# thethomasboyer/PhenDiff

Measured on NVIDIA B200. Metric: images/sec, DDIM invert+regenerate 128x128 100 steps, higher is better.
Workload: dtype fp16

## Files before the change

include/phendiff_b200.h:

```cpp
#ifndef PHENDIFF_B200_H
#define PHENDIFF_B200_H

#include <stddef.h>
#include <stdint.h>

#ifdef __cplusplus
extern "C" {
#endif

typedef struct pd_unet pd_unet_t;
typedef struct pd_train pd_train_t;
typedef void* pd_stream_t;

enum { PD_PREC_FP32 = 0, PD_PREC_BF16 = 1, PD_PREC_FP16 = 2 };
enum { PD_PRED_EPSILON = 0, PD_PRED_SAMPLE = 1, PD_PRED_V = 2 };
#define PD_MAX_BLOCKS 8

typedef struct pd_unet_config {
    int32_t in_channels;
    int32_t out_channels;
    int32_t n_blocks;
    int32_t block_out_channels[PD_MAX_BLOCKS];
    int32_t down_attn[PD_MAX_BLOCKS];
    int32_t up_attn[PD_MAX_BLOCKS];
// ... 76 lines not shown
                       pd_stream_t stream);
int pd_train_launch_count(pd_train_t* t, int64_t* n);

int pd_train_forward(pd_train_t* t, const float* params, const float* x, const float* timesteps, const int64_t* labels, float* model_out,
                     pd_stream_t stream);
int pd_train_backward_input(pd_train_t* t, const float* d_model_out, float* d_input, pd_stream_t stream);
int pd_guidance_lp_grad(const pd_step_coeffs_t* step, const float* x, const float* model_out, const float* ref, int32_t batch, int64_t per,
                        float p, float* scratch, float* losses, float* d_model_out, float* d_x, pd_stream_t stream);
#define PD_ADAMW_SCRATCH_FLOATS 1185
int pd_adamw_step(float* params, const float* grads, float* exp_avg, float* exp_avg_sq, float* ema, int64_t n, float lr, float beta1,
                  float beta2, float eps, float weight_decay, int32_t step, float max_grad_norm, float ema_decay, float* scratch,
                  float* grad_norm_out, pd_stream_t stream);

int pd_unet_launch_count(pd_unet_t* h, int64_t* n);
int pd_unet_plan_info(pd_unet_t* h, int32_t* microbatch, int32_t* tc_layers, int32_t* simt_layers, int32_t* ops);

enum { PD_CLS_CONV_TC = 0, PD_CLS_CONV_SIMT, PD_CLS_GN, PD_CLS_ATTN, PD_CLS_EMBED, PD_CLS_CONV_IN, PD_CLS_CONV_OUT,
       PD_CLS_UPSAMPLE, PD_CLS_COUNT };
int pd_unet_profile_begin(pd_unet_t* h, int32_t every_n, int32_t max_samples);
int pd_unet_profile_end(pd_unet_t* h, int32_t* samples);
int pd_unet_profile_query(pd_unet_t* h, int32_t cls, double* ms, int64_t* launches, double* flops);
int pd_unet_profile_op(pd_unet_t* h, int32_t idx, const char** name, int32_t* cls, double* ms, int32_t* samples, double* flops);

int pd_test_conv(int32_t use_tc, int32_t dtype, int32_t n, int32_t h, int32_t w, int32_t c1, int32_t c2,
                 int32_t cout, int32_t ksize, int32_t stride, int32_t pad, const void* x1, const void* x2,
                 const float* weight, const float* bias, const float* addvec, const void* residual,
                 const void* sc1, const void* sc2, int32_t csc1, int32_t csc2, const float* sc_w, float out_scale,
                 void* out, pd_stream_t stream);
typedef struct pd_test_conv_args {
    int32_t impl, dtype, n, h, w, c1, c2, cout, ksize, stride, pad, upsample, mode, stats_cw, csc1, csc2;
    const void *x1, *x2;
    const float *weight, *bias, *addvec;
    const int32_t* addvec_row;
    const void* residual;
    const void *sc1, *sc2;
    const float* sc_w;
    float out_scale;
    void* out;
    double* stats_out;
    float* model_out;
    float* x_t;
    const pd_step_coeffs_t* step;
} pd_test_conv_args_t;
int pd_test_conv_ex(const pd_test_conv_args_t* args, pd_stream_t stream);
int pd_test_gn_conv(int32_t dtype, int32_t n, int32_t h, int32_t w, int32_t c1, int32_t c2, int32_t cout, int32_t groups, float eps,
                    const void* x1, const void* x2, const float* gamma, const float* beta, const float* weight, const float* bias,
                    const float* addvec, const void* residual, const void* sc1, const void* sc2, int32_t csc1, int32_t csc2,
                    const float* sc_w, float out_scale, void* out, double* stats_out, pd_stream_t stream);
int pd_test_groupnorm(int32_t dtype, int32_t n, int32_t hw, int32_t c1, int32_t c2, int32_t groups, float eps,
                      int32_t do_silu, const void* x1, const void* x2, const float* gamma, const float* beta,
                      void* out, pd_stream_t stream);
int pd_test_attention(int32_t use_mma, int32_t dtype, int32_t n, int32_t s, int32_t c, int32_t d, const void* qkv,
                      void* out, pd_stream_t stream);

#ifdef __cplusplus
}
#endif
#endif
```

phendiff_b200/_lib.py:

```python
from __future__ import annotations

import ctypes as C
import os
from pathlib import Path

_HERE = Path(__file__).resolve().parent
LIB_PATH = _HERE / "libphendiff_b200.so"

PD_PREC_FP32, PD_PREC_BF16, PD_PREC_FP16 = 0, 1, 2
PD_PRED = {"epsilon": 0, "sample": 1, "v_prediction": 2}
PD_MAX_BLOCKS = 8


class UnetConfig(C.Structure):
    _fields_ = [
        ("in_channels", C.c_int32), ("out_channels", C.c_int32), ("n_blocks", C.c_int32),
        ("block_out_channels", C.c_int32 * PD_MAX_BLOCKS),
        ("down_attn", C.c_int32 * PD_MAX_BLOCKS), ("up_attn", C.c_int32 * PD_MAX_BLOCKS),
        ("layers_per_block", C.c_int32), ("attention_head_dim", C.c_int32), ("norm_num_groups", C.c_int32),
        ("norm_eps", C.c_float), ("num_class_embeds", C.c_int32), ("flip_sin_to_cos", C.c_int32),
        ("freq_shift", C.c_float), ("downsample_padding", C.c_int32), ("mid_block_scale_factor", C.c_float),
        ("add_attention", C.c_int32), ("precision", C.c_int32), ("max_microbatch", C.c_int32),
        ("conv_impl", C.c_int32), ("attn_impl", C.c_int32),
    ]
# ... 13 lines not shown
                + [(n, C.c_void_p) for n in ("x1", "x2", "weight", "bias", "addvec", "addvec_row", "residual", "sc1", "sc2", "sc_w")]
                + [("out_scale", C.c_float)]
                + [(n, C.c_void_p) for n in ("out", "stats_out", "model_out", "x_t", "step")])


_P = C.c_void_p
_SIGNATURES = {
    "pd_last_error": (C.c_char_p, []),
    "pd_version": (C.c_int, []),
    "pd_unet_create": (C.c_int, [C.POINTER(UnetConfig), C.POINTER(_P)]),
    "pd_unet_destroy": (C.c_int, [_P]),
    "pd_unet_num_params": (C.c_int, [_P, C.POINTER(C.c_int32)]),
    "pd_unet_param_info": (C.c_int, [_P, C.c_int32, C.POINTER(C.c_char_p), C.POINTER(C.c_int32), C.POINTER(C.c_int64 * 4)]),
    "pd_unet_load_weight": (C.c_int, [_P, C.c_char_p, _P, C.POINTER(C.c_int64), C.c_int32]),
    "pd_unet_finalize": (C.c_int, [_P, _P]),
    "pd_unet_time_embed_dim": (C.c_int, [_P, C.POINTER(C.c_int32)]),
    "pd_unet_plan": (C.c_int, [_P, C.c_int32, C.c_int32, C.c_int32, C.POINTER(C.c_size_t)]),
    "pd_unet_bind_workspace": (C.c_int, [_P, _P, C.c_size_t]),
    "pd_unet_forward": (C.c_int, [_P, _P, _P, _P, _P, _P, _P]),
    "pd_ddim_step": (C.c_int, [C.POINTER(StepCoeffs), _P, _P, _P, _P, _P, C.c_int64, _P]),
    "pd_axpby_per_sample": (C.c_int, [_P, _P, _P, _P, _P, C.c_int32, C.c_int64, _P]),
    "pd_cfg_combine": (C.c_int, [_P, _P, _P, C.c_int32, _P, C.c_int32, C.c_int64, _P]),
    "pd_denorm_nhwc": (C.c_int, [_P, _P, C.c_int32, C.c_int32, C.c_int32, C.c_int32, _P]),
    "pd_ddib_transfer": (C.c_int, [_P, _P, _P, _P, C.POINTER(StepCoeffs), C.c_int32, C.c_int32, _P]),
    "pd_unet_plan_guided": (C.c_int, [_P, C.c_int32, C.c_int32, C.c_int32, C.POINTER(C.c_size_t)]),
    "pd_cfg_transfer": (C.c_int, [_P, _P, _P, _P, C.c_int32, C.POINTER(StepCoeffs), C.c_int32, _P]),
    "pd_train_create": (C.c_int, [_P, C.c_int32, C.c_int32, C.c_int32, C.POINTER(_P)]),
    "pd_train_destroy": (C.c_int, [_P]),
    "pd_train_set_precision": (C.c_int, [_P, C.c_int32]),
    "pd_train_tc_counts": (C.c_int, [_P, C.POINTER(C.c_int64), C.POINTER(C.c_int64)]),
    "pd_train_num_params_flat": (C.c_int, [_P, C.POINTER(C.c_int64)]),
    "pd_train_param_offset": (C.c_int, [_P, C.c_int32, C.POINTER(C.c_int64)]),
    "pd_train_workspace_bytes": (C.c_int, [_P, C.POINTER(C.c_size_t)]),
    "pd_train_bind": (C.c_int, [_P, _P, C.c_size_t]),
    "pd_train_step_grad": (C.c_int, [_P] * 11),
    "pd_train_launch_count": (C.c_int, [_P, C.POINTER(C.c_int64)]),
    "pd_train_forward": (C.c_int, [_P] * 7),
    "pd_train_backward_input": (C.c_int, [_P] * 4),
    "pd_guidance_lp_grad": (C.c_int, [C.POINTER(StepCoeffs), _P, _P, _P, C.c_int32, C.c_int64, C.c_float, _P, _P, _P, _P, _P]),
    "pd_adamw_step": (C.c_int, [_P, _P, _P, _P, _P, C.c_int64, C.c_float, C.c_float, C.c_float, C.c_float, C.c_float, C.c_int32,
                                 C.c_float, C.c_float, _P, _P, _P]),
    "pd_debug_pair_kernel_launches": (C.c_longlong, []),
    "pd_unet_launch_count": (C.c_int, [_P, C.POINTER(C.c_int64)]),
    "pd_unet_plan_info": (C.c_int, [_P, C.POINTER(C.c_int32), C.POINTER(C.c_int32), C.POINTER(C.c_int32), C.POINTER(C.c_int32)]),
    "pd_unet_profile_begin": (C.c_int, [_P, C.c_int32, C.c_int32]),
    "pd_unet_profile_end": (C.c_int, [_P, C.POINTER(C.c_int32)]),
    "pd_unet_profile_query": (C.c_int, [_P, C.c_int32, C.POINTER(C.c_double), C.POINTER(C.c_int64), C.POINTER(C.c_double)]),
    "pd_unet_profile_op": (C.c_int, [_P, C.c_int32, C.POINTER(C.c_char_p), C.POINTER(C.c_int32), C.POINTER(C.c_double), C.POINTER(C.c_int32), C.POINTER(C.c_double)]),
    "pd_test_conv": (C.c_int, [C.c_int32] * 11 + [_P, _P, _P, _P, _P, _P, _P, _P, C.c_int32, C.c_int32, _P, C.c_float, _P, _P]),
    "pd_test_conv_ex": (C.c_int, [C.POINTER(TestConvArgs), _P]),
    "pd_test_gn_conv": (C.c_int, [C.c_int32] * 8 + [C.c_float] + [_P] * 10 + [C.c_int32, C.c_int32, _P, C.c_float, _P, _P, _P]),
    "pd_test_groupnorm": (C.c_int, [C.c_int32] * 6 + [C.c_float, C.c_int32, _P, _P, _P, _P, _P, _P]),
    "pd_test_attention": (C.c_int, [C.c_int32] * 6 + [_P, _P, _P]),
}

EXPORTED_SYMBOLS = tuple(_SIGNATURES)

_lib = None


class PhenDiffB200Error(RuntimeError):
    pass


def lib():
    global _lib
    if _lib is None:
        path = os.environ.get("PHENDIFF_B200_LIB", str(LIB_PATH))
        if not os.path.exists(path):
            raise PhenDiffB200Error(
                f"{path} not found: build it with `python -c 'import __graft_entry__ as g; g.build()'` "
                "(or phendiff_b200/csrc/build.sh). phendiff_b200 has no CPU or PyTorch fallback.")
        l = C.CDLL(path)
        for name, (res, args) in _SIGNATURES.items():
            fn = getattr(l, name)
            fn.restype = res
            fn.argtypes = args
        _lib = l
    return _lib


def check(rc: int):
    if rc != 0:
        msg = lib().pd_last_error()
        raise PhenDiffB200Error(msg.decode() if msg else f"phendiff_b200 error code {rc}")


def ptr(t):
    return None if t is None else C.c_void_p(t.data_ptr())


def current_stream():
    import torch

    return C.c_void_p(torch.cuda.current_stream().cuda_stream)


def require_cuda(t, what: str):
    if not t.is_cuda:
        raise PhenDiffB200Error(
            f"{what} must be a CUDA tensor: phendiff_b200 is the B200 path and has no CPU fallback (got device {t.device})")
```

phendiff_b200/csrc/pd_api.cu:

```cuda
#include "pd_model.h"

namespace pd {

static thread_local std::string g_err;
void set_error(const std::string& m) { g_err = m; }

}

using namespace pd;


namespace pd {

static Param* add_param(pd_unet* m, const std::string& name, std::vector<int64_t> shape) {
    auto p = std::make_unique<Param>();
    p->name = name;
    p->shape = shape;
    p->numel = 1;
    for (auto s : shape) p->numel *= (size_t)s;
    Param* r = p.get();
    m->by_name[name] = r;
    m->params.push_back(std::move(p));
    return r;
}
// ... 1226 lines not shown
    return rc;
}

int pd_test_conv(int32_t use_tc, int32_t dt, int32_t n, int32_t h, int32_t w, int32_t c1, int32_t c2, int32_t cout,
                 int32_t ksize, int32_t stride, int32_t pad, const void* x1, const void* x2, const float* weight,
                 const float* bias, const float* addvec, const void* residual, const void* sc1, const void* sc2,
                 int32_t csc1, int32_t csc2, const float* sc_w, float out_scale, void* out, pd_stream_t stream) {
    pd_test_conv_args_t a;
    memset(&a, 0, sizeof(a));
    a.impl = use_tc; a.dtype = dt; a.n = n; a.h = h; a.w = w; a.c1 = c1; a.c2 = c2; a.cout = cout; a.ksize = ksize;
    a.stride = stride; a.pad = pad; a.x1 = x1; a.x2 = x2; a.weight = weight; a.bias = bias; a.addvec = addvec;
    a.residual = residual; a.sc1 = sc1; a.sc2 = sc2; a.csc1 = csc1; a.csc2 = csc2; a.sc_w = sc_w; a.out_scale = out_scale;
    a.out = out;
    return pd_test_conv_ex(&a, stream);
}

int pd_test_groupnorm(int32_t dt, int32_t n, int32_t hw, int32_t c1, int32_t c2, int32_t groups, float eps,
                      int32_t do_silu, const void* x1, const void* x2, const float* gamma, const float* beta, void* out,
                      pd_stream_t stream) {
    cudaStream_t s = (cudaStream_t)stream;
    PD_REQUIRE(groups > 0 && (c1 + c2) % groups == 0, "channels not divisible by groups");
    int cw = 4;
    while (cw > 1 && (((c1 + c2) / groups) % cw != 0 || c1 % cw != 0)) cw >>= 1;
    double* stats = nullptr;
    const size_t n1 = (size_t)n * (c1 / cw) * 2, n2 = (size_t)n * (c2 / cw) * 2;
    PD_CHECK_CUDA(cudaMalloc((void**)&stats, (n1 + n2 + 2) * sizeof(double)));
    PD_CHECK_CUDA(cudaMemsetAsync(stats, 0, (n1 + n2 + 2) * sizeof(double), s));
    GNArgs ga{};
    ga.x1 = x1; ga.x2 = x2; ga.C1 = c1; ga.C2 = c2; ga.N = n; ga.HW = hw; ga.groups = groups; ga.eps = eps; ga.gamma = gamma;
    ga.beta = beta; ga.silu = do_silu; ga.stats1 = stats; ga.stats2 = c2 ? stats + n1 : nullptr; ga.stats_cw = cw; ga.out = out;
    int rc = launch_gn_chunk_stats(dt, x1, n, hw, c1, cw, stats, s);
    if (!rc && c2) rc = launch_gn_chunk_stats(dt, x2, n, hw, c2, cw, stats + n1, s);
    if (!rc) rc = launch_gn_apply(dt, dt == 0, ga, s);
    cudaError_t e = cudaStreamSynchronize(s);
    cudaFree(stats);
    if (!rc && e != cudaSuccess) { set_error(std::string("groupnorm kernel failed: ") + cudaGetErrorString(e)); rc = 2; }
    return rc;
}

int pd_test_attention(int32_t use_mma, int32_t dt, int32_t n, int32_t s_len, int32_t c, int32_t d, const void* qkv,
                      void* out, pd_stream_t stream) {
    cudaStream_t s = (cudaStream_t)stream;
    int rc;
    if (use_mma) {
        rc = launch_attention_mma(dt, qkv, n, s_len, c, d, use_mma >= 2 ? PD_ATTN_QFOLD : 1.0f, out, s, use_mma >= 3 ? use_mma - 1 : 0);
    } else {
        rc = launch_attention_simt(dt, dt == 0, qkv, n, s_len, c, d, out, s);
    }
    cudaError_t e = cudaStreamSynchronize(s);
    if (!rc && e != cudaSuccess) { set_error(std::string("attention kernel failed: ") + cudaGetErrorString(e)); rc = 2; }
    return rc;
}

}
```

phendiff_b200/csrc/pd_attn_common.cuh:

```cuda
#pragma once
#include "pd_kernels.h"
#include <type_traits>

namespace pd {

__device__ __forceinline__ float ex2(float x) {
    float y;
    asm("ex2.approx.ftz.f32 %0, %1;" : "=f"(y) : "f"(x));
    return y;
}
__device__ __forceinline__ float ex2_poly(float x) {
    x = fminf(fmaxf(x, -100.0f), 128.0f);
    const float t = x + 12582912.0f;
    const float f = x - (t - 12582912.0f);
    float p = 0.05508868396282196f;
    p = fmaf(p, f, 0.24260404706001282f);
    p = fmaf(p, f, 0.6932762265205383f);
    p = fmaf(p, f, 0.9999289512634277f);
    return __int_as_float(__float_as_int(p) + (__float_as_int(t) << 23));
}
__device__ __forceinline__ uint32_t h2op_add(uint32_t a, uint32_t b) { uint32_t d; asm("add.rn.f16x2 %0, %1, %2;" : "=r"(d) : "r"(a), "r"(b)); return d; }
__device__ __forceinline__ uint32_t h2op_sub(uint32_t a, uint32_t b) { uint32_t d; asm("sub.rn.f16x2 %0, %1, %2;" : "=r"(d) : "r"(a), "r"(b)); return d; }
__device__ __forceinline__ uint32_t h2op_mul(uint32_t a, uint32_t b) { uint32_t d; asm("mul.rn.f16x2 %0, %1, %2;" : "=r"(d) : "r"(a), "r"(b)); return d; }
__device__ __forceinline__ uint32_t h2op_fma(uint32_t a, uint32_t b, uint32_t c) { uint32_t d; asm("fma.rn.f16x2 %0, %1, %2, %3;" : "=r"(d) : "r"(a), "r"(b), "r"(c)); return d; }
__device__ __forceinline__ uint32_t h2op_min(uint32_t a, uint32_t b) { uint32_t d; asm("min.f16x2 %0, %1, %2;" : "=r"(d) : "r"(a), "r"(b)); return d; }
__device__ __forceinline__ uint32_t h2op_max(uint32_t a, uint32_t b) { uint32_t d; asm("max.f16x2 %0, %1, %2;" : "=r"(d) : "r"(a), "r"(b)); return d; }

__device__ __forceinline__ uint32_t ex2_pair_h2(float xa, float xb) {
    uint32_t x = pack_f16x2(xa, xb);
    x = h2op_min(h2op_max(x, 0xCB80CB80u ), 0x4C004C00u );
    const uint32_t w = h2op_add(x, 0x640F640Fu );
    const uint32_t f = h2op_sub(x, h2op_sub(w, 0x640F640Fu));
    uint32_t p = h2op_fma(0x2B0D2B0Du , f, 0x33C333C3u );
    p = h2op_fma(p, f, 0x398C398Cu );
    p = h2op_fma(p, f, 0x3C003C00u );
    return h2op_mul(p, w * 1024u + (0u - 0x64006400u * 1024u));
}

template <typename T> __device__ __forceinline__ uint32_t ex2_pair_poly(float xa, float xb);
template <> __device__ __forceinline__ uint32_t ex2_pair_poly<f16>(float xa, float xb) { return ex2_pair_h2(xa, xb); }
template <> __device__ __forceinline__ uint32_t ex2_pair_poly<bf16>(float xa, float xb) { return pack_bf16x2(ex2_poly(xa), ex2_poly(xb)); }


}
```

phendiff_b200/csrc/pd_attn_mma.cu:

```cuda
#include "pd_attn_common.cuh"

namespace pd {

constexpr int AT_WARPS = 8;
constexpr int AT_MAXS = 1024;

template <typename T>
__device__ __forceinline__ void mma_16x8x8(float c[4], uint32_t a0, uint32_t a1, uint32_t b0) {
    if (std::is_same<T, bf16>::value)
        asm volatile("mma.sync.aligned.m16n8k8.row.col.f32.bf16.bf16.f32 {%0,%1,%2,%3}, {%4,%5}, {%6}, {%0,%1,%2,%3};"
                     : "+f"(c[0]), "+f"(c[1]), "+f"(c[2]), "+f"(c[3])
                     : "r"(a0), "r"(a1), "r"(b0));
    else
        asm volatile("mma.sync.aligned.m16n8k8.row.col.f32.f16.f16.f32 {%0,%1,%2,%3}, {%4,%5}, {%6}, {%0,%1,%2,%3};"
                     : "+f"(c[0]), "+f"(c[1]), "+f"(c[2]), "+f"(c[3])
                     : "r"(a0), "r"(a1), "r"(b0));
}
template <typename T>
__device__ __forceinline__ void mma_16x8x16(float c[4], uint32_t a0, uint32_t a1, uint32_t a2, uint32_t a3, uint32_t b0,
                                            uint32_t b1) {
    if (std::is_same<T, bf16>::value)
        asm volatile(
            "mma.sync.aligned.m16n8k16.row.col.f32.bf16.bf16.f32 {%0,%1,%2,%3}, {%4,%5,%6,%7}, {%8,%9}, {%0,%1,%2,%3};"
            : "+f"(c[0]), "+f"(c[1]), "+f"(c[2]), "+f"(c[3])
// ... 346 lines not shown
    if (variant < 0) {
        const char* e = getenv("PHENDIFF_B200_ATTN_KERNEL");
        variant = !e ? 6 : ((e[0] == 'v' && e[1] == '2') ? 2 : ((e[0] == 't' && e[1] == 'c') ? (e[2] == '3' ? 6 : (e[2] == '2' ? 5 : 4)) : 3));
        const char* pe = getenv("PHENDIFF_B200_ATTN_POLYPAIRS");
        polyv = pe ? atoi(pe) : -1;
    }
    const size_t smem = (size_t)S * 32;
    const int var = force_variant ? force_variant : variant;
    if (var == 2 || smem > 200 * 1024) return launch_attention_chunked(dt, qkv, N, S, C, d, AH_SL / qfold, out, s);
    const bool tc3 = var == 6 && S % 128 == 0 && attention_tc3_supported(S, C) && fabsf(AH_SL / qfold - 1.0f) < 1e-6f;
    if (tc3 || ((var == 4 || var == 5) && S % 128 == 0 && attention_tc_smem_bytes(S) <= 110 * 1024)) {
        static uint8_t* flags_dev[PD_MAX_DEVICES] = {nullptr};
        static size_t flags_cap_dev[PD_MAX_DEVICES] = {0};
        uint8_t*& flags = flags_dev[pd_cur_dev()];
        size_t& flags_cap = flags_cap_dev[pd_cur_dev()];
        const size_t need = (size_t)N * (C / 8) * (S >> 7) * 4;
        if (need > flags_cap) {
            if (flags) PD_CHECK_CUDA(cudaFree(flags));
            PD_CHECK_CUDA(cudaMalloc(&flags, need));
            flags_cap = need;
        }
        const int tc_pp = polyv < 0 ? (dt == DT_F16 ? 4 : 2) : polyv;
        int rc = tc3 ? launch_attention_tc3(dt, qkv, N, S, C, out, flags, tc_pp, s)
                 : (var == 5 ? launch_attention_tc2(dt, qkv, N, S, C, AH_SL / qfold, out, flags, tc_pp, s)
                             : launch_attention_tc(dt, qkv, N, S, C, AH_SL / qfold, out, flags, tc_pp, s));
        if (rc) return rc;
        dim3 grid(1, C / 8, N);
        PD_DISPATCH_HALF(dt, T, (launch_head<T, 0x0000u>(qkv, N, S, C, AH_SL / qfold, out, grid, smem, s, flags)));
        PD_CHECK_CUDA(cudaGetLastError());
        return 0;
    }
    const float qmul = AH_SL / qfold;
    const int heads = C / 8;
    int split = 1;
    while (split < 8 && (size_t)heads * N * split < 1184 && (S >> 4) / (split * 2) >= AH_WARPS) split *= 2;
    dim3 grid(split, heads, N);
    int pp = polyv;
    if (pp < 0) pp = (dt == DT_F16) ? 6 : 4;
#define PD_AH(MASK) PD_DISPATCH_HALF(dt, T, (launch_head<T, MASK>(qkv, N, S, C, qmul, out, grid, smem, s)))
    switch (pp) {
        case 0: PD_AH(0x0000u); break;
        case 4: PD_AH(0x4242u); break;
        case 6: PD_AH(0x6262u); break;
        case 7: PD_AH(0x6662u); break;
        case 10: PD_AH(0xE6E6u); break;
        case 12: PD_AH(0xEEEEu); break;
        default: PD_AH(0x6666u); break;
    }
#undef PD_AH
    PD_CHECK_CUDA(cudaGetLastError());
    return 0;
}

}
```

phendiff_b200/csrc/pd_attn_tc3.cu:

```cuda
#include "pd_attn_common.cuh"
#include "pd_tc_common.cuh"

namespace pd {

constexpr int A3_NWG = 3;
__host__ __device__ constexpr int a3_threads(int sp) { return 128 + 128 * A3_NWG * sp; }
constexpr int A3_TMEM_COLS = 512;
constexpr int A3_WG_COLS = 160;
constexpr int A3_KT = 64;

struct A3Params {
    CUtensorMap tm;
    int S, C, heads, items, tok_box;
    void* out;
    uint8_t* flags;
    int swap_k, swap_mn;
    int nws;
};

__device__ __forceinline__ void a3_mma_ts(uint32_t d_tmem, uint32_t a_tmem, uint64_t b_desc, uint32_t idesc, uint32_t accumulate) {
    asm volatile(
        "{\n\t.reg .pred p;\n\tsetp.ne.b32 p, %4, 0;\n\t"
        "tcgen05.mma.cta_group::1.kind::f16 [%0], [%1], %2, %3, p;\n\t}\n" ::"r"(d_tmem),
        "r"(a_tmem), "l"(b_desc), "r"(idesc), "r"(accumulate)
// ... 8 lines not shown
        : "memory");
}
__device__ __forceinline__ void a3_st_wait() { asm volatile("tcgen05.wait::st.sync.aligned;" ::: "memory"); }
__device__ __forceinline__ void a3_ld_x16(uint32_t taddr, uint32_t (&r)[16]) {
    asm volatile(
        "tcgen05.ld.sync.aligned.32x32b.x16.b32 "
        "{%0, %1, %2, %3, %4, %5, %6, %7, %8, %9, %10, %11, %12, %13, %14, %15}, [%16];"
        : "=r"(r[0]), "=r"(r[1]), "=r"(r[2]), "=r"(r[3]), "=r"(r[4]), "=r"(r[5]), "=r"(r[6]), "=r"(r[7]),
          "=r"(r[8]), "=r"(r[9]), "=r"(r[10]), "=r"(r[11]), "=r"(r[12]), "=r"(r[13]), "=r"(r[14]), "=r"(r[15])
        : "r"(taddr));
}

__device__ __forceinline__ bool a3_try_wait_hint(uint64_t* bar, uint32_t parity, uint32_t ns) {
    uint32_t ok;
    asm volatile(
        "{\n\t.reg .pred P;\n\tmbarrier.try_wait.parity.shared::cta.b64 P, [%1], %2, %3;\n\tselp.b32 %0, 1, 0, P;\n\t}\n"
        : "=r"(ok) : "r"(smem_u32(bar)), "r"(parity), "r"(ns) : "memory");
    return ok != 0;
}
__device__ __forceinline__ void a3_wait(uint64_t* bar, uint32_t parity) {
    if (a3_try_wait_hint(bar, parity, 2000u)) return;
    const long long t0 = clock64();
    for (;;) {
#pragma unroll 1
        for (int k = 0; k < 64; ++k)
            if (a3_try_wait_hint(bar, parity, 2000u)) return;
        if (clock64() - t0 > 4000000000LL) {
            printf("phendiff_b200: attention_tc3 mbarrier wait timed out (block %d thread %d)\n", blockIdx.x, threadIdx.x);
            __trap();
        }
    }
}

__device__ __forceinline__ void a3_wait_warp(uint64_t* bar, uint32_t parity) {
    if (elect_one()) {
        bool ok = mbar_test(bar, parity);
#pragma unroll 1
        for (int k = 0; k < 4096 && !ok; ++k) ok = mbar_test(bar, parity);
        if (!ok) a3_wait(bar, parity);
    }
    __syncwarp();
}

__device__ __forceinline__ void a3_spin(uint32_t bar, uint32_t parity) {
    asm volatile(
        "{\n\t.reg .pred P1;\n\tA3_WAIT:\n\tmbarrier.try_wait.parity.shared::cta.b64 P1, [%0], %1;\n\t@P1 bra A3_DONE;\n\tbra A3_WAIT;\n\tA3_DONE:\n\t}\n"
        ::"r"(bar), "r"(parity) : "memory");
}

__device__ __forceinline__ uint64_t a3_desc(uint32_t addr, uint32_t lbo, uint32_t sbo) {
    return (uint64_t)((addr & 0x3FFFFu) >> 4) | ((uint64_t)((lbo >> 4) & 0x3FFFu) << 16) | ((uint64_t)((sbo >> 4) & 0x3FFFu) << 32) |
           ((uint64_t)1 << 46);
}
template <typename T, int N, bool B_MN> __device__ __forceinline__ constexpr uint32_t a3_idesc() {
    constexpr uint32_t fmt = std::is_same<T, bf16>::value ? 1u : 0u;
    return (1u << 4) | (fmt << 7) | (fmt << 10) | ((B_MN ? 1u : 0u) << 16) | ((uint32_t)(N >> 3) << 17) | ((uint32_t)(128 >> 4) << 24);
}
template <typename T> __device__ __forceinline__ uint32_t a3_pack_raw(T lo, T hi) {
    return (uint32_t)(*reinterpret_cast<const uint16_t*>(&lo)) | ((uint32_t)(*reinterpret_cast<const uint16_t*>(&hi)) << 16);
}

template <typename T, int PP, bool SUB>
__device__ __forceinline__ void a3_exp32(const uint32_t (&s)[32], float sub, uint32_t (&p)[16]) {
#pragma unroll
    for (int r = 0; r < 16; ++r) {
        float x0 = __uint_as_float(s[2 * r]), x1 = __uint_as_float(s[2 * r + 1]);
        if (SUB) { x0 -= sub; x1 -= sub; }
        if (PP == 9) { p[r] = pack2<T>(fmaf(fabsf(x0), 1e-4f, 1e-3f), fmaf(fabsf(x1), 1e-4f, 1e-3f)); continue; }
        const bool poly = PP > 0 && ((r * PP) & 7) < PP;
        p[r] = poly ? ex2_pair_poly<T>(x0, x1) : pack2<T>(ex2(x0), ex2(x1));
    }
}

template <typename T, int PP, int SP>
__global__ void __launch_bounds__(a3_threads(SP), 1) attention_tc3_kernel(const __grid_constant__ A3Params p) {
    constexpr int A3_THREADS = a3_threads(SP);
    extern __shared__ uint8_t a3_smem_raw[];
    uint8_t* smem = reinterpret_cast<uint8_t*>((reinterpret_cast<uintptr_t>(a3_smem_raw) + 127) & ~(uintptr_t)127);
    const int S = p.S, C = p.C;
    const uint32_t opb = (uint32_t)S * 16u;
    const uint32_t stage_bytes = 3u * opb;
    uint8_t* sm_kaug = smem + 2 * (size_t)stage_bytes;
    uint8_t* sm_vaug = sm_kaug + 1024;
    uint8_t* sm_zero = sm_vaug + 256;
    uint8_t* sm_qaug = sm_zero + 2048;
    uint64_t* bars = reinterpret_cast<uint64_t*>(sm_qaug + A3_NWG * 2048);
    uint64_t* qkv_full = bars;
    uint64_t* qkv_empty = bars + 2;
    uint64_t* sfull = bars + 4;
    uint64_t* pready = bars + 10;
    uint64_t* ofull = bars + 16;
    uint64_t* oread = bars + 22;
    uint64_t* qmready = bars + 28;
    uint32_t* tmem_slot = reinterpret_cast<uint32_t*>(bars + 31);
    float* sm_xmax = reinterpret_cast<float*>(bars + 32);

    const int warp = threadIdx.x >> 5, lane = threadIdx.x & 31;
    const int nqt = S >> 7, ntl = S / A3_KT;
#ifdef A3_TRACE
    __shared__ long long tr_soft[40][5];
    __shared__ long long tr_iss[40][4];
    __shared__ long long tr_w[40][4][2];
    __shared__ long long tr_mma[40][6];
#endif
    const int my_items = (p.items - (int)blockIdx.x + (int)gridDim.x - 1) / (int)gridDim.x;
    const int total_T = my_items * nqt;

    if (warp == 1 && lane == 0) {
        for (int i = 0; i < 2; ++i) { mbar_init(&qkv_full[i], 1); mbar_init(&qkv_empty[i], (uint32_t)nqt); }
        for (int i = 0; i < A3_NWG * 2; ++i) { mbar_init(&sfull[i], 1); mbar_init(&pready[i], 4 * SP); mbar_init(&ofull[i], 1); mbar_init(&oread[i], 4); }
        for (int i = 0; i < A3_NWG; ++i) mbar_init(&qmready[i], 4);
        fence_barrier_init();
    }
    if (warp == 0 && lane == 0) prefetch_tmap(&p.tm);
    if (warp == 2) {
        tmem_alloc(tmem_slot, A3_TMEM_COLS);
        tmem_relinquish();
    }
    {
        const T one = from_f<T>(1.0f), zero = from_f<T>(0.0f);
        const uint32_t ones2 = a3_pack_raw<T>(one, one), one1 = a3_pack_raw<T>(one, zero);
        for (int i = threadIdx.x; i < 64; i += A3_THREADS) *reinterpret_cast<uint4*>(sm_kaug + i * 16) = make_uint4(ones2, 0u, 0u, 0u);
        for (int i = threadIdx.x; i < 16; i += A3_THREADS) *reinterpret_cast<uint4*>(sm_vaug + i * 16) = make_uint4(one1, 0u, 0u, 0u);
        for (int i = threadIdx.x; i < 128 * (1 + A3_NWG); i += A3_THREADS) *reinterpret_cast<uint4*>(sm_zero + i * 16) = make_uint4(0u, 0u, 0u, 0u);
    }
    fence_proxy_async();
    tc_fence_before();
    __syncthreads();
    tc_fence_after();
    const uint32_t tmem_base = *tmem_slot;

    if (warp == 0) {
        if (lane == 0) {
            for (int it = 0; it < my_items; ++it) {
                const int stage = it & 1;
                a3_wait(&qkv_empty[stage], (uint32_t)(((it >> 1) & 1) ^ 1));
                const int item = (int)blockIdx.x + it * (int)gridDim.x;
                const int n = item / p.heads, head = item - n * p.heads;
                mbar_arrive_expect_tx(&qkv_full[stage], stage_bytes);
                uint8_t* dst = smem + (size_t)stage * stage_bytes;
                for (int which = 0; which < 3; ++which)
                    for (int t0 = 0; t0 < S; t0 += p.tok_box)
                        tma_load_3d(&p.tm, &qkv_full[stage], dst + (size_t)which * opb + (size_t)t0 * 16, which * C + head * 8, t0, n);
            }
        }
    } else if (warp < 4) {
        const int g = __shfl_sync(0xffffffffu, warp, 0) - 1;
        const int nTg = (g >= 0 && g < p.nws && total_T > g) ? (total_T - g + p.nws - 1) / p.nws : 0;
        if (nTg > 0) {
            constexpr uint32_t idS = a3_idesc<T, A3_KT, false>(), idPV = a3_idesc<T, 16, true>();
            constexpr uint32_t HI_K = (128u >> 4) | (1u << 14);
            const uint32_t sm0 = smem_u32(smem), kaug = smem_u32(sm_kaug), vaug = smem_u32(sm_vaug), zaug = smem_u32(sm_zero);
            const uint32_t qaug = smem_u32(sm_qaug) + (uint32_t)g * 2048u;
            const uint32_t tS = tmem_base + (uint32_t)(g * A3_WG_COLS), tO = tS + 128u;
            const uint32_t bar_sfull = smem_u32(&sfull[g * 2]), bar_pready = smem_u32(&pready[g * 2]);
            const uint32_t bar_ofull = smem_u32(&ofull[g * 2]), bar_oread = smem_u32(&oread[g * 2]);
            const uint32_t bar_qm = smem_u32(&qmready[g]), bar_full = smem_u32(qkv_full), bar_empty = smem_u32(qkv_empty);
            auto lo_k = [](uint32_t start, uint32_t aug) { return ((start & 0x3FFFFu) >> 4) | ((((aug - start) >> 4) & 0x3FFFu) << 16); };
            auto mma_S = [&](int buf, uint32_t a_lo, uint32_t b_lo) {
                if (elect_one()) {
                    umma_f16kind(tS + (uint32_t)(buf * 64), desc64(HI_K, a_lo), desc64(HI_K, b_lo), idS, 0u);
                    umma_commit_addr(bar_sfull + buf * 8);
                }
                __syncwarp();
            };
            auto mma_PV = [&](int buf, uint32_t d, uint32_t v_lo, uint32_t v_hi, bool first, bool last, uint32_t ob, uint32_t eb) {
                if (elect_one()) {
                    const uint32_t a0 = tS + (uint32_t)(buf * 64);
#pragma unroll
                    for (int kk = 0; kk < 4; ++kk)
                        a3_mma_ts(d, a0 + (uint32_t)(32 * (kk >> 1) + 8 * (kk & 1)), desc64(v_hi - 16u * kk, v_lo + 16u * kk), idPV, (!first || kk) ? 1u : 0u);
                    if (last) { umma_commit_addr(ob); umma_commit_addr(eb); }
                }
                __syncwarp();
            };
            int it = 0, qt = g, items_seen = 0;
            while (qt >= nqt) { qt -= nqt; ++it; }
            a3_spin(bar_full + (it & 1) * 8, (uint32_t)(it >> 1) & 1u);
            items_seen = it + 1;
            tc_fence_after();
            uint32_t stage0 = sm0 + (uint32_t)(it & 1) * stage_bytes;
            uint32_t qs = stage0 + (uint32_t)qt * 2048u;
            mma_S(0, lo_k(qs, zaug), lo_k(stage0 + opb, kaug));
            for (int k = 0; k < nTg; ++k) {
                const uint32_t a_aug = lo_k(qs, qaug);
                uint32_t b_lo = lo_k(stage0 + opb + A3_KT * 16u, kaug);
                const uint32_t vs0 = stage0 + 2u * opb;
                uint32_t v_lo = ((vs0 & 0x3FFFFu) >> 4) | ((128u >> 4) << 16);
                uint32_t v_hi = (((vaug - vs0) >> 4) & 0x3FFFu) | (1u << 14);
                const uint32_t d = tO + (uint32_t)(16 * (k & 1));
                const uint32_t ob = bar_ofull + (k & 1) * 8, eb = bar_empty + (it & 1) * 8;
                int it_n = it, qt_n = qt + p.nws;
                while (qt_n >= nqt) { qt_n -= nqt; ++it_n; }
                const bool has_next = k + 1 < nTg;
                const uint32_t stage_n = sm0 + (uint32_t)(it_n & 1) * stage_bytes;
                const uint32_t qs_n = stage_n + (uint32_t)qt_n * 2048u;
                a3_spin(bar_qm, (uint32_t)k & 1u);
                tc_fence_after();
                mma_S(1, a_aug, b_lo);
                b_lo += 64u - (64u << 16);
                if (k >= 2) a3_spin(bar_oread + (k & 1) * 8, (uint32_t)((k >> 1) - 1) & 1u);
                const uint32_t par0 = (uint32_t)(k * (ntl >> 1)) & 1u;
#pragma unroll 1
// ... 50 lines not shown
                it = it_n; qt = qt_n; stage0 = stage_n; qs = qs_n;
            }
        }

    } else if (warp >= 4) {
        const int sw = warp - 4;
        const int g = sw / (4 * SP), half = (sw >> 2) % SP, wq = warp & 3;
        const int row = wq * 32 + lane;
        constexpr int NC = 64 / SP;
        const uint32_t lane_base = tmem_base + ((uint32_t)(wq * 32) << 16) + (uint32_t)(g * A3_WG_COLS);
        uint8_t* my_qaug = sm_qaug + g * 2048 + row * 16;
        T* out = reinterpret_cast<T*>(p.out);
        const int nTg = (g < p.nws && total_T > g) ? (total_T - g + p.nws - 1) / p.nws : 0;
        auto finish_qtile = [&](int k) {
            const int Tq = g + p.nws * k, it = Tq / nqt, qt = Tq - it * nqt;
            const int item = (int)blockIdx.x + it * (int)gridDim.x;
            const int n = item / p.heads, head = item - n * p.heads;
            a3_wait(&ofull[g * 2 + (k & 1)], (uint32_t)(k >> 1) & 1u);
            tc_fence_after();
            uint32_t o[16];
            a3_ld_x16(lane_base + (uint32_t)(128 + 16 * (k & 1)), o);
            tmem_ld_wait();
            tc_fence_before();
            __syncwarp();
            if (lane == 0) mbar_arrive(&oread[g * 2 + (k & 1)]);
            const float l = __uint_as_float(o[8]);
            bool bad = !(fabsf(l) <= 3.0e38f) || !(l > 0.f);
            float v[8];
            const float inv = 1.0f / l;
#pragma unroll
            for (int c = 0; c < 8; ++c) {
                const float oc = __uint_as_float(o[c]);
                bad = bad || !(fabsf(oc) <= 3.0e38f);
                v[c] = oc * inv;
            }
            store8(out + ((size_t)n * S + qt * 128 + row) * C + head * 8, v);
            const bool anybad = __any_sync(0xffffffffu, bad);
            if (lane == 0) p.flags[(((size_t)n * p.heads + head) * nqt + qt) * 4 + wq] = anybad ? 1 : 0;
        };
        int s = 0;
        for (int k = 0; k < nTg; ++k) {
            float m = 0.f;
            for (int j = 0; j < ntl; ++j, ++s) {
                const int buf = s & 1;
                a3_wait(&sfull[g * 2 + buf], (uint32_t)(s >> 1) & 1u);
                tc_fence_after();
#ifdef A3_TRACE
                const bool trc = blockIdx.x == 0 && warp == 4 && lane == 0 && s >= 20 && s < 60;
                if (trc) tr_soft[s - 20][0] = clock64();
                const bool trw = blockIdx.x == 0 && g == 0 && lane == 0 && s >= 20 && s < 60;
                if (trw) tr_w[s - 20][wq][0] = clock64();
#endif
                const uint32_t ts = lane_base + (uint32_t)(buf * 64 + half * NC);
                uint32_t s0[32], p0[16];
                tmem_ld_32x32b_x32(ts, s0);
                tmem_ld_wait();
                if (SP == 1) {
                    uint32_t s1[32], p1[16];
                    tmem_ld_32x32b_x32(ts + 32u, s1);
                    if (j == 0) {
                        tmem_ld_wait();
                        float mx = __uint_as_float(s0[0]);
#pragma unroll
                        for (int c = 1; c < 32; ++c) mx = fmaxf(mx, __uint_as_float(s0[c]));
#pragma unroll
                        for (int c = 0; c < 32; ++c) mx = fmaxf(mx, __uint_as_float(s1[c]));
                        m = mx;
                        const T mh = from_f<T>(-m);
                        const T ml = from_f<T>(-m - to_f(mh));
                        *reinterpret_cast<uint4*>(my_qaug) = make_uint4(a3_pack_raw<T>(mh, ml), 0u, 0u, 0u);
                        fence_proxy_async();
                        __syncwarp();
                        if (lane == 0) mbar_arrive(&qmready[g]);
                        a3_exp32<T, PP, true>(s0, m, p0);
                        a3_st_x16(ts, p0);
                        a3_exp32<T, PP, true>(s1, m, p1);
                        a3_st_x16(ts + 32u, p1);
                    } else {
                        a3_exp32<T, PP, false>(s0, 0.f, p0);
                        a3_st_x16(ts, p0);
                        tmem_ld_wait();
#ifdef A3_TRACE
                        if (trc) tr_soft[s - 20][1] = clock64();
#endif
                        a3_exp32<T, PP, false>(s1, 0.f, p1);
                        a3_st_x16(ts + 32u, p1);
#ifdef A3_TRACE
                        if (trc) tr_soft[s - 20][2] = clock64();
#endif
                    }
                } else {
                    if (j == 0) {
                        float mx = __uint_as_float(s0[0]);
#pragma unroll
                        for (int c = 1; c < 32; ++c) mx = fmaxf(mx, __uint_as_float(s0[c]));
                        sm_xmax[(g * 2 + half) * 128 + row] = mx;
                        asm volatile("bar.sync %0, %1;" ::"r"(1 + g), "r"(128 * SP) : "memory");
                        m = fmaxf(mx, sm_xmax[(g * 2 + (half ^ 1)) * 128 + row]);
                        if (half == 0) {
                            const T mh = from_f<T>(-m);
                            const T ml = from_f<T>(-m - to_f(mh));
                            *reinterpret_cast<uint4*>(my_qaug) = make_uint4(a3_pack_raw<T>(mh, ml), 0u, 0u, 0u);
                            fence_proxy_async();
                            __syncwarp();
                            if (lane == 0) mbar_arrive(&qmready[g]);
                        }
                        a3_exp32<T, PP, true>(s0, m, p0);
                    } else {
                        a3_exp32<T, PP, false>(s0, 0.f, p0);
                    }
                    a3_st_x16(ts, p0);
                }
                a3_st_wait();
#ifdef A3_TRACE
                if (trc) tr_soft[s - 20][3] = clock64();
#endif
                tc_fence_before();
                __syncwarp();
                if (lane == 0) mbar_arrive(&pready[g * 2 + buf]);
#ifdef A3_TRACE
                if (trc) tr_soft[s - 20][4] = clock64();
                if (trw) tr_w[s - 20][wq][1] = clock64();
#endif
                if (j == 0 && k >= 1 && half == 0) finish_qtile(k - 1);
            }
        }
        if (nTg > 0 && half == 0) finish_qtile(nTg - 1);
    }
    tc_fence_before();
    __syncthreads();
#ifdef A3_TRACE
    if (blockIdx.x == 0 && threadIdx.x == 0) {
        for (int i = 0; i < 40; ++i) {
            printf("step %2d soft(w4..7): wake %lld %lld %lld %lld arrive %lld %lld %lld %lld || iss: top %lld spin-done %lld (+%lld) PV-done +%lld S-done +%lld\n", 20 + i,
                   tr_w[i][0][0] - tr_soft[0][0], tr_w[i][1][0] - tr_soft[0][0], tr_w[i][2][0] - tr_soft[0][0], tr_w[i][3][0] - tr_soft[0][0],
                   tr_w[i][0][1] - tr_soft[0][0], tr_w[i][1][1] - tr_soft[0][0], tr_w[i][2][1] - tr_soft[0][0], tr_w[i][3][1] - tr_soft[0][0],
                   tr_iss[i][3] - tr_soft[0][0], tr_iss[i][0] - tr_soft[0][0], tr_iss[i][0] - tr_iss[i][3], tr_iss[i][1] - tr_iss[i][0], tr_iss[i][2] - tr_iss[i][1]);
        }
    }
#endif
    if (warp == 2) {
        tc_fence_after();
        tmem_dealloc(tmem_base, A3_TMEM_COLS);
    }
}

size_t attention_tc3_smem_bytes(int S) { return (size_t)2 * 3 * S * 16 + 1024 + 256 + 2048 + A3_NWG * 2048 + 32 * 8 + A3_NWG * 2 * 128 * 4 + 128; }

// ... 55 lines not shown
```

phendiff_b200/csrc/pd_kernels.h:

```cpp
#pragma once
#include "pd_common.cuh"
#include "../../include/phendiff_b200.h"

namespace pd {

struct EmbedArgs {
    const float* timesteps;
    float t_scalar;
    const int64_t* labels;
    const float* class_emb;
    const float *w1, *b1;
    const float *w2, *b2;
    const float* class_table;
    int B, C0, D, ncls, flip;
    float shift;
    float* emb_act;
    int dedupe;
    int32_t* row_idx;
    int cfg_pairs;
};
inline int embed_rows(const EmbedArgs& a) { return a.dedupe ? a.ncls + ((a.cfg_pairs > 0 || a.ncls == 0) ? 1 : 0) : a.B; }

struct CfgEpi {
    const float* uncond;
// ... 15 lines not shown
    void* out;
};
int launch_gn_chunk_stats(int dt, const void* x, int N, int HW, int C, int cw, double* stats, cudaStream_t s);
int launch_gn_apply(int dt, bool precise, const GNArgs& a, cudaStream_t s);
int launch_gn_coef(const GNArgs& a, float2* coef, cudaStream_t s);

struct ConvArgs {
    const void* x1; const void* x2;
    int C1, C2, N, H, W, Cout, ksize, stride, pad, Ho, Wo;
    const float* w;
    const float* bias;
    const float* addvec;
    const int32_t* addvec_row;
    int addvec_stride;
    const void* residual;
    float out_scale;
    void* out;
};
int launch_conv_simt(int dt, const ConvArgs& a, cudaStream_t s);

int launch_conv_in(int dt, const float* x, const float* w , const float* bias, int N, int Cin, int H,
                   int W, int Cout, void* out, cudaStream_t s, int n_src = 0);
struct ConvOutArgs {
    const void* act;
    const float* w;
    const float* bias;
    int N, H, W, Cin, Cout;
    float* model_out;
    float* x;
    const pd_step_coeffs_t* step;
    int img_begin, img_count;
    CfgEpi cfg;
};
int launch_conv_out(int dt, const ConvOutArgs& a, cudaStream_t s);

int launch_upsample2x(int dt, const void* x, int N, int H, int W, int C, void* out, cudaStream_t s);
int launch_im2col_in(int dt, const float* x, int N, int Cin, int H, int W, void* out, cudaStream_t s, int n_src = 0);

int launch_attention_simt(int dt, bool precise, const void* qkv, int N, int S, int C, int d, void* out,
                          cudaStream_t s);
int launch_attention_generic(int dt, bool precise, const void* qkv, int N, int S, int C, int d, void* out, cudaStream_t s);
constexpr float PD_ATTN_QFOLD = 0.35355339059327373f * 1.4426950408889634f;
int launch_attention_mma(int dt, const void* qkv, int N, int S, int C, int d, float qfold, void* out, cudaStream_t s,
                         int force_variant = 0);
size_t attention_tc_smem_bytes(int S);
int attention_mma_launches(int S);
int launch_attention_tc(int dt, const void* qkv, int N, int S, int C, float qmul, void* out, uint8_t* flags, int poly_pairs,
                        cudaStream_t s);
int launch_attention_tc2(int dt, const void* qkv, int N, int S, int C, float qmul, void* out, uint8_t* flags, int poly_pairs,
                        cudaStream_t s);

bool attention_tc3_supported(int S, int C);
int launch_attention_tc3(int dt, const void* qkv, int N, int S, int C, void* out, uint8_t* flags, int poly_pairs, cudaStream_t s);

#ifdef __CUDACC__
__device__ __forceinline__ float ddim_update(const pd_step_coeffs_t& c, float x, float m, float noise, float* x0_out) {
    float x0, e;
    if (c.pred_type == PD_PRED_EPSILON) {
        x0 = (x - c.sqrt_beta * m) / c.sqrt_alpha;
        e = m;
    } else if (c.pred_type == PD_PRED_SAMPLE) {
        x0 = m;
        e = (x - c.sqrt_alpha * x0) / c.sqrt_beta;
    } else {
        x0 = c.sqrt_alpha * x - c.sqrt_beta * m;
        e = c.sqrt_alpha * m + c.sqrt_beta * x;
    }
    if (c.clip) x0 = (x0 < -c.clip_range) ? -c.clip_range : ((x0 > c.clip_range) ? c.clip_range : x0);
    if (c.use_clipped_model_output) e = (x - c.sqrt_alpha * x0) / c.sqrt_beta;
    float out = c.sqrt_alpha_next * x0 + c.dir_coef * e;
    if (c.sigma != 0.f) out += c.sigma * noise;
    if (x0_out) *x0_out = x0;
    return out;
}
#endif
int launch_ddim_step(const pd_step_coeffs_t& c, const float* x, const float* m, const float* noise, float* x_out,
                     float* x0_out, int64_t n, cudaStream_t s);
int launch_axpby(const float* a, const float* b, const float* ca, const float* cb, float* out, int B, int64_t per,
                 cudaStream_t s);
int launch_cfg(const float* cond, const float* uncond, const float* w, int eqn, float* out, int B, int64_t per,
               cudaStream_t s);
int launch_denorm(const float* x, float* out, int B, int C, int H, int W, cudaStream_t s);

int launch_relayout_simt(const float* w, int O, int I, int k, float* out, cudaStream_t s);
int launch_relayout_tc(int dt, const float* w, int O, int I, int k, void* out, int ktot, int koff, cudaStream_t s);
int launch_relayout_convout(const float* w, int O, int I, float* out, cudaStream_t s);
int launch_cast_half(int dt, const float* x, void* out, int64_t n, cudaStream_t s);

struct ConvTcPlan;
enum { TC_MODE_STD = 0, TC_MODE_DDIM = 1 };
struct ConvTcDesc {
    int dt;
    const void* x; int C;
    const void* x2; int C2;
    const float2* gn_coef;
    int N, H, W, ksize, stride, pad, Ho, Wo, Cout;
    int upsample;
    const void* sc1; int Csc1;
    const void* sc2; int Csc2;
    const void* wmat;
    const float* bias;
    const float* addvec; int addvec_stride;
    const int32_t* addvec_row;
    const void* residual;
    float out_scale;
    void* out;
// ... 22 lines not shown
```

Measured before the change: 15.50.

## Accumulate attention scores in fp16 TMEM and run softmax exp in packed half2

For fp16, the tcgen05 attention kernel now sets the instruction descriptor to produce fp16 S accumulators. It loads them with packed 16-bit TMEM loads (16 registers instead of 32) and computes row max, max subtraction and exp2 directly in f16x2, using either the polynomial or the MUFU ex2.approx.f16x2 path. This is meant to halve TMEM load traffic and register pressure and to cut the conversion and packing work in the softmax. The cost is reduced precision in the QK^T scores and the max subtraction. A test entry point for comparing the two ex2 routes is also added.

```diff
diff --git a/include/phendiff_b200.h b/include/phendiff_b200.h
--- a/include/phendiff_b200.h
+++ b/include/phendiff_b200.h
@@ -152,6 +152,7 @@
                       void* out, pd_stream_t stream);
 int pd_test_attention(int32_t use_mma, int32_t dtype, int32_t n, int32_t s, int32_t c, int32_t d, const void* qkv,
                       void* out, pd_stream_t stream);
+int pd_test_ex2_h2(int32_t route, int32_t n, const void* x, void* y, pd_stream_t stream);
 
 #ifdef __cplusplus
 }
diff --git a/phendiff_b200/_lib.py b/phendiff_b200/_lib.py
--- a/phendiff_b200/_lib.py
+++ b/phendiff_b200/_lib.py
@@ -89,6 +89,7 @@
     "pd_test_gn_conv": (C.c_int, [C.c_int32] * 8 + [C.c_float] + [_P] * 10 + [C.c_int32, C.c_int32, _P, C.c_float, _P, _P, _P]),
     "pd_test_groupnorm": (C.c_int, [C.c_int32] * 6 + [C.c_float, C.c_int32, _P, _P, _P, _P, _P, _P]),
     "pd_test_attention": (C.c_int, [C.c_int32] * 6 + [_P, _P, _P]),
+    "pd_test_ex2_h2": (C.c_int, [C.c_int32, C.c_int32, _P, _P, _P]),
 }
 
 EXPORTED_SYMBOLS = tuple(_SIGNATURES)
diff --git a/phendiff_b200/csrc/pd_api.cu b/phendiff_b200/csrc/pd_api.cu
--- a/phendiff_b200/csrc/pd_api.cu
+++ b/phendiff_b200/csrc/pd_api.cu
@@ -1302,4 +1302,12 @@
     return rc;
 }
 
-}
+int pd_test_ex2_h2(int32_t route, int32_t n, const void* x, void* y, pd_stream_t stream) {
+    cudaStream_t s = (cudaStream_t)stream;
+    int rc = launch_ex2_h2_test(x, y, n, route, s);
+    cudaError_t e = cudaStreamSynchronize(s);
+    if (!rc && e != cudaSuccess) { set_error(std::string("ex2_h2 test kernel failed: ") + cudaGetErrorString(e)); rc = 2; }
+    return rc;
+}
+
+}
diff --git a/phendiff_b200/csrc/pd_attn_common.cuh b/phendiff_b200/csrc/pd_attn_common.cuh
--- a/phendiff_b200/csrc/pd_attn_common.cuh
+++ b/phendiff_b200/csrc/pd_attn_common.cuh
@@ -26,8 +26,7 @@
 __device__ __forceinline__ uint32_t h2op_min(uint32_t a, uint32_t b) { uint32_t d; asm("min.f16x2 %0, %1, %2;" : "=r"(d) : "r"(a), "r"(b)); return d; }
 __device__ __forceinline__ uint32_t h2op_max(uint32_t a, uint32_t b) { uint32_t d; asm("max.f16x2 %0, %1, %2;" : "=r"(d) : "r"(a), "r"(b)); return d; }
 
-__device__ __forceinline__ uint32_t ex2_pair_h2(float xa, float xb) {
-    uint32_t x = pack_f16x2(xa, xb);
+__device__ __forceinline__ uint32_t ex2_h2(uint32_t x) {
     x = h2op_min(h2op_max(x, 0xCB80CB80u ), 0x4C004C00u );
     const uint32_t w = h2op_add(x, 0x640F640Fu );
     const uint32_t f = h2op_sub(x, h2op_sub(w, 0x640F640Fu));
@@ -36,6 +35,12 @@
     p = h2op_fma(p, f, 0x3C003C00u );
     return h2op_mul(p, w * 1024u + (0u - 0x64006400u * 1024u));
 }
+__device__ __forceinline__ uint32_t ex2_h2_mufu(uint32_t x) {
+    uint32_t y;
+    asm("ex2.approx.f16x2 %0, %1;" : "=r"(y) : "r"(x));
+    return y;
+}
+__device__ __forceinline__ uint32_t ex2_pair_h2(float xa, float xb) { return ex2_h2(pack_f16x2(xa, xb)); }
 
 template <typename T> __device__ __forceinline__ uint32_t ex2_pair_poly(float xa, float xb);
 template <> __device__ __forceinline__ uint32_t ex2_pair_poly<f16>(float xa, float xb) { return ex2_pair_h2(xa, xb); }
diff --git a/phendiff_b200/csrc/pd_attn_mma.cu b/phendiff_b200/csrc/pd_attn_mma.cu
--- a/phendiff_b200/csrc/pd_attn_mma.cu
+++ b/phendiff_b200/csrc/pd_attn_mma.cu
@@ -422,4 +422,18 @@
     return 0;
 }
 
-}
+__global__ void ex2_h2_test_kernel(const uint32_t* __restrict__ x, uint32_t* __restrict__ y, int n2, int route) {
+    for (int i = blockIdx.x * blockDim.x + threadIdx.x; i < n2; i += gridDim.x * blockDim.x) y[i] = route ? ex2_h2_mufu(x[i]) : ex2_h2(x[i]);
+}
+
+int launch_ex2_h2_test(const void* x, void* y, int n, int route, cudaStream_t s) {
+    PD_REQUIRE(n >= 0 && n % 2 == 0, "ex2_h2 test: n must be even (packed pairs)");
+    PD_REQUIRE(route == 0 || route == 1, "ex2_h2 test: route is 0 (polynomial) or 1 (MUFU)");
+    const int n2 = n / 2;
+    if (n2 == 0) return 0;
+    ex2_h2_test_kernel<<<std::min((n2 + 255) / 256, 1024), 256, 0, s>>>((const uint32_t*)x, (uint32_t*)y, n2, route);
+    PD_CHECK_CUDA(cudaGetLastError());
+    return 0;
+}
+
+}
diff --git a/phendiff_b200/csrc/pd_attn_tc3.cu b/phendiff_b200/csrc/pd_attn_tc3.cu
--- a/phendiff_b200/csrc/pd_attn_tc3.cu
+++ b/phendiff_b200/csrc/pd_attn_tc3.cu
@@ -84,23 +84,65 @@
     return (uint64_t)((addr & 0x3FFFFu) >> 4) | ((uint64_t)((lbo >> 4) & 0x3FFFu) << 16) | ((uint64_t)((sbo >> 4) & 0x3FFFu) << 32) |
            ((uint64_t)1 << 46);
 }
-template <typename T, int N, bool B_MN> __device__ __forceinline__ constexpr uint32_t a3_idesc() {
+template <typename T, int N, bool B_MN, bool D16> __device__ __forceinline__ constexpr uint32_t a3_idesc() {
     constexpr uint32_t fmt = std::is_same<T, bf16>::value ? 1u : 0u;
-    return (1u << 4) | (fmt << 7) | (fmt << 10) | ((B_MN ? 1u : 0u) << 16) | ((uint32_t)(N >> 3) << 17) | ((uint32_t)(128 >> 4) << 24);
+    return ((D16 ? 0u : 1u) << 4) | (fmt << 7) | (fmt << 10) | ((B_MN ? 1u : 0u) << 16) | ((uint32_t)(N >> 3) << 17) |
+           ((uint32_t)(128 >> 4) << 24);
 }
 template <typename T> __device__ __forceinline__ uint32_t a3_pack_raw(T lo, T hi) {
     return (uint32_t)(*reinterpret_cast<const uint16_t*>(&lo)) | ((uint32_t)(*reinterpret_cast<const uint16_t*>(&hi)) << 16);
 }
 
+template <typename T> __host__ __device__ constexpr bool a3_s16() { return std::is_same<T, f16>::value; }
+template <typename T> __host__ __device__ constexpr int a3_sregs() { return a3_s16<T>() ? 16 : 32; }
+
+__device__ __forceinline__ void a3_ld_x16_pack(uint32_t taddr, uint32_t (&r)[16]) {
+    asm volatile(
+        "tcgen05.ld.sync.aligned.32x32b.x16.pack::16b.b32 "
+        "{%0, %1, %2, %3, %4, %5, %6, %7, %8, %9, %10, %11, %12, %13, %14, %15}, [%16];"
+        : "=r"(r[0]), "=r"(r[1]), "=r"(r[2]), "=r"(r[3]), "=r"(r[4]), "=r"(r[5]), "=r"(r[6]), "=r"(r[7]),
+          "=r"(r[8]), "=r"(r[9]), "=r"(r[10]), "=r"(r[11]), "=r"(r[12]), "=r"(r[13]), "=r"(r[14]), "=r"(r[15])
+        : "r"(taddr));
+}
+template <typename T> __device__ __forceinline__ void a3_ld_s(uint32_t taddr, uint32_t (&s)[a3_sregs<T>()]) {
+    if constexpr (a3_s16<T>()) a3_ld_x16_pack(taddr, s);
+    else tmem_ld_32x32b_x32(taddr, s);
+}
+template <typename T> __device__ __forceinline__ float a3_rowmax(const uint32_t (&s)[a3_sregs<T>()]) {
+    if constexpr (a3_s16<T>()) {
+        uint32_t m = s[0];
+#pragma unroll
+        for (int c = 1; c < 16; ++c) m = h2op_max(m, s[c]);
+        const __half2 h = *reinterpret_cast<const __half2*>(&m);
+        return fmaxf(__low2float(h), __high2float(h));
+    } else {
+        float mx = __uint_as_float(s[0]);
+#pragma unroll
+        for (int c = 1; c < 32; ++c) mx = fmaxf(mx, __uint_as_float(s[c]));
+        return mx;
+    }
+}
+
 template <typename T, int PP, bool SUB>
-__device__ __forceinline__ void a3_exp32(const uint32_t (&s)[32], float sub, uint32_t (&p)[16]) {
+__device__ __forceinline__ void a3_exp32(const uint32_t (&s)[a3_sregs<T>()], float sub, uint32_t (&p)[16]) {
+    if constexpr (a3_s16<T>()) {
+        const uint32_t m2 = pack_f16x2(sub, sub);
 #pragma unroll
-    for (int r = 0; r < 16; ++r) {
-        float x0 = __uint_as_float(s[2 * r]), x1 = __uint_as_float(s[2 * r + 1]);
-        if (SUB) { x0 -= sub; x1 -= sub; }
-        if (PP == 9) { p[r] = pack2<T>(fmaf(fabsf(x0), 1e-4f, 1e-3f), fmaf(fabsf(x1), 1e-4f, 1e-3f)); continue; }
-        const bool poly = PP > 0 && ((r * PP) & 7) < PP;
-        p[r] = poly ? ex2_pair_poly<T>(x0, x1) : pack2<T>(ex2(x0), ex2(x1));
+        for (int r = 0; r < 16; ++r) {
+            const uint32_t x = SUB ? h2op_sub(s[r], m2) : s[r];
+            if (PP == 9) { p[r] = h2op_fma(x & 0x7FFF7FFFu, 0x068E068Eu, 0x14191419u); continue; }
+            const bool poly = PP > 0 && ((r * PP) & 7) < PP;
+            p[r] = poly ? ex2_h2(x) : ex2_h2_mufu(x);
+        }
+    } else {
+#pragma unroll
+        for (int r = 0; r < 16; ++r) {
+            float x0 = __uint_as_float(s[2 * r]), x1 = __uint_as_float(s[2 * r + 1]);
+            if (SUB) { x0 -= sub; x1 -= sub; }
+            if (PP == 9) { p[r] = pack2<T>(fmaf(fabsf(x0), 1e-4f, 1e-3f), fmaf(fabsf(x1), 1e-4f, 1e-3f)); continue; }
+            const bool poly = PP > 0 && ((r * PP) & 7) < PP;
+            p[r] = poly ? ex2_pair_poly<T>(x0, x1) : pack2<T>(ex2(x0), ex2(x1));
+        }
     }
 }
 
@@ -180,7 +222,7 @@
         const int g = __shfl_sync(0xffffffffu, warp, 0) - 1;
         const int nTg = (g >= 0 && g < p.nws && total_T > g) ? (total_T - g + p.nws - 1) / p.nws : 0;
         if (nTg > 0) {
-            constexpr uint32_t idS = a3_idesc<T, A3_KT, false>(), idPV = a3_idesc<T, 16, true>();
+            constexpr uint32_t idS = a3_idesc<T, A3_KT, false, a3_s16<T>()>(), idPV = a3_idesc<T, 16, true, false>();
             constexpr uint32_t HI_K = (128u >> 4) | (1u << 14);
             const uint32_t sm0 = smem_u32(smem), kaug = smem_u32(sm_kaug), vaug = smem_u32(sm_vaug), zaug = smem_u32(sm_zero);
             const uint32_t qaug = smem_u32(sm_qaug) + (uint32_t)g * 2048u;
@@ -337,20 +379,16 @@
                 if (trw) tr_w[s - 20][wq][0] = clock64();
 #endif
                 const uint32_t ts = lane_base + (uint32_t)(buf * 64 + half * NC);
-                uint32_t s0[32], p0[16];
-                tmem_ld_32x32b_x32(ts, s0);
+                constexpr int SR = a3_sregs<T>();
+                uint32_t s0[SR], p0[16];
+                a3_ld_s<T>(ts, s0);
                 tmem_ld_wait();
                 if (SP == 1) {
-                    uint32_t s1[32], p1[16];
-                    tmem_ld_32x32b_x32(ts + 32u, s1);
+                    uint32_t s1[SR], p1[16];
+                    a3_ld_s<T>(ts + 32u, s1);
                     if (j == 0) {
                         tmem_ld_wait();
-                        float mx = __uint_as_float(s0[0]);
-#pragma unroll
-                        for (int c = 1; c < 32; ++c) mx = fmaxf(mx, __uint_as_float(s0[c]));
-#pragma unroll
-                        for (int c = 0; c < 32; ++c) mx = fmaxf(mx, __uint_as_float(s1[c]));
-                        m = mx;
+                        m = fmaxf(a3_rowmax<T>(s0), a3_rowmax<T>(s1));
                         const T mh = from_f<T>(-m);
                         const T ml = from_f<T>(-m - to_f(mh));
                         *reinterpret_cast<uint4*>(my_qaug) = make_uint4(a3_pack_raw<T>(mh, ml), 0u, 0u, 0u);
@@ -376,9 +414,7 @@
                     }
                 } else {
                     if (j == 0) {
-                        float mx = __uint_as_float(s0[0]);
-#pragma unroll
-                        for (int c = 1; c < 32; ++c) mx = fmaxf(mx, __uint_as_float(s0[c]));
+                        const float mx = a3_rowmax<T>(s0);
                         sm_xmax[(g * 2 + half) * 128 + row] = mx;
                         asm volatile("bar.sync %0, %1;" ::"r"(1 + g), "r"(128 * SP) : "memory");
                         m = fmaxf(mx, sm_xmax[(g * 2 + (half ^ 1)) * 128 + row]);
diff --git a/phendiff_b200/csrc/pd_kernels.h b/phendiff_b200/csrc/pd_kernels.h
--- a/phendiff_b200/csrc/pd_kernels.h
+++ b/phendiff_b200/csrc/pd_kernels.h
@@ -91,6 +91,7 @@
 
 bool attention_tc3_supported(int S, int C);
 int launch_attention_tc3(int dt, const void* qkv, int N, int S, int C, void* out, uint8_t* flags, int poly_pairs, cudaStream_t s);
+int launch_ex2_h2_test(const void* x, void* y, int n, int route, cudaStream_t s);
 
 #ifdef __CUDACC__
 __device__ __forceinline__ float ddim_update(const pd_step_coeffs_t& c, float x, float m, float noise, float* x0_out) {
```

After: 15.85 (median of 6 runs). +2.3%, better.
